# dnbaker/dashing

Measured on AMD Instinct MI355X. Metric: genome-pairs/sec, all-pairs HLL Jaccard (Ertl-MLE), N=10000 p=14, higher is better.
Workload: dtype u8/u32 popcount + f64 estimator; 1 GPU; BASELINE configs[2]: 10000 synthetic sketches, p=14 (16384 B each), all-pairs dist on MI355X; n_sketches=10000, p=14, k=31, estimator=ERTL_MLE

## Files before the change

dashing_amd/csrc/abi.hip:

```cpp
#include <algorithm>
#include <cstdlib>
#include <cstring>
#include <new>

#include "ctx.h"

using namespace dsh;

extern "C" {

const char *dsh_backend_name(void) { return "hip:gfx950"; }

int dsh_abi_version(void) { return DSH_ABI_VERSION; }

int dsh_device_count(void)
{
    int n = 0;
    if (hipGetDeviceCount(&n) != hipSuccess) return 0;
    return n;
}

static void release_ctx(dsh_ctx *c)
{
    (void)hipSetDevice(c->device);
// ... 476 lines not shown
    if (!c || !nparts_out) return DSH_EINVAL;
    const uint32_t k = (uint32_t)c->part_ready_ms.size();
    *nparts_out = k;
    if (k > cap && (ready_ms || floats)) return DSH_EINVAL;
    for (uint32_t q = 0; q < k; ++q) {
        if (ready_ms) ready_ms[q] = c->part_ready_ms[q];
        if (floats) floats[q] = c->part_floats[q];
    }
    return DSH_OK;
}

int dsh_finalize_phase_cycles(dsh_ctx *c, uint64_t *out16)
{
    if (!c || !out16) return DSH_EINVAL;
    int rc = bind(c);
    if (rc) return rc;
    if (!c->phase_cyc.ptr) return fail(c, DSH_ESTATE, "no call with the option finalize_timing yet");
    HIPCHK(c, hipStreamSynchronize(c->stream));
    HIPCHK(c, hipMemcpy(out16, c->phase_cyc.ptr, 16 * sizeof(uint64_t), hipMemcpyDeviceToHost));
    return DSH_OK;
}

int dsh_get_info(dsh_ctx *c, const char *name, int64_t *out)
{
    if (!c || !name || !out) return DSH_EINVAL;
    if (!std::strcmp(name, "planes")) *out = c->lay.P;
    else if (!std::strcmp(name, "vlo")) *out = c->lay.vlo;
    else if (!std::strcmp(name, "vhi")) *out = c->lay.vhi;
    else if (!std::strcmp(name, "threshold")) *out = c->lay.pbase + (int64_t)c->lay.P;
    else if (!std::strcmp(name, "pbase")) *out = c->lay.pbase;
    else if (!std::strcmp(name, "host_layout_us")) *out = (int64_t)c->host_layout_us;
    else if (!std::strcmp(name, "host_lists_us")) *out = (int64_t)c->host_lists_us;
    else if (!std::strcmp(name, "host_keys_wait_us")) *out = (int64_t)c->host_keys_wait_us;
    else if (!std::strcmp(name, "emax")) *out = c->emax;
    else if (!std::strcmp(name, "elow")) *out = c->elow;
    else if (!std::strcmp(name, "kc")) *out = c->kc;
    else if (!std::strcmp(name, "pair_groups")) *out = c->pair_groups;
    else if (!std::strcmp(name, "pair_round")) *out = c->pp.band_round.empty() ? 0 : c->pp.band_round[0];
    else if (!std::strcmp(name, "tile")) *out = kTile;
    else if (!std::strcmp(name, "parts_done")) *out = c->parts_done;
    else if (!std::strcmp(name, "parts_signalled")) *out = c->parts_signalled ? 1 : 0;
    else if (!std::strcmp(name, "sketch_kernel_us")) *out = (int64_t)(c->sketch_ms * 1000.0);
    else if (!std::strcmp(name, "fastx_decode_us")) *out = (int64_t)(c->fastx_ms * 1000.0);
    else if (!std::strcmp(name, "xch_recv_gated")) *out = c->xch.recv_gated ? 1 : 0;
    else if (!std::strcmp(name, "stats_route")) *out = c->gs.route_last;
    else if (!std::strcmp(name, "linkage_route")) *out = c->lk.route_last;
    else if (!std::strcmp(name, "mst_rounds")) *out = c->mst.rounds_last;
    else if (!std::strcmp(name, "mst_band_us")) *out = (int64_t)(c->mst.band_ms * 1000.0);
    else if (!std::strcmp(name, "place_kernel_us")) *out = (int64_t)(c->xch.place_ms * 1000.0);
    else if (!std::strcmp(name, "whatif_mfma")) {
#ifdef DSH_WHATIF_MFMA
        *out = 1;
#else
        *out = 0;
#endif
    }
    else if (!std::strcmp(name, "npad")) *out = c->lay.Npad;
    else if (!std::strcmp(name, "kpad")) *out = c->Kpad;
    else if (!std::strcmp(name, "cum_bytes")) *out = c->cum_bytes;
    else if (!std::strcmp(name, "sorted")) *out = c->lay.sorted;
    else if (!std::strcmp(name, "ncols")) *out = (int64_t)c->lay.ncols;
    else if (!std::strcmp(name, "lockstep")) *out = c->planes_valid && use_lockstep(c) ? 1 : 0;
    else if (!std::strcmp(name, "tiles")) *out = (int64_t)c->pp.T.size();
    else if (!std::strcmp(name, "bands")) *out = (int64_t)c->last_bands;
    else if (!std::strcmp(name, "items")) *out = (int64_t)c->pp.items.size();
    else if (!std::strcmp(name, "frag_items")) {
// ... 121 lines not shown
```

dashing_amd/csrc/ctx.h:

```cpp
#pragma once
#include <hip/hip_runtime.h>
#include <rccl/rccl.h>

#include <cstdarg>
#include <cstdio>
#include <cstdlib>
#include <deque>
#include <string>
#include <vector>

#include "../../include/dashing_hip.h"
#include "kernels.h"
#include "plan.h"

struct NoCopy {
    NoCopy() = default;
    NoCopy(const NoCopy &) = delete;
    NoCopy &operator=(const NoCopy &) = delete;
};

struct DevBuf : NoCopy {
    void *ptr = nullptr;
    size_t cap = 0;
    ~DevBuf() { release(); }
// ... 119 lines not shown
    Event ev_filled[2];
    Event ev_drained[2];
    bool drained_pending[2] = {false, false};
    unsigned out_turn = 0;
    std::deque<Event> tickets;
    uint64_t ticket_next = 0;
    Event ev_first_tiles;
    bool pass_from_zero = false;
    DevBuf hist;
    Event ev_keys;
    DevBuf cidx_rec, cidx_ent;
    uint32_t nbuckets = 0, ent_stride = 0;
    DevBuf colS_n, colS_key, colS_card, colS_th, colS_rl;
    uint32_t rl_stride = 0;
    dsh::plan::Layout lay;
    bool lay_built = false;
    dsh::plan::PairPlan pp;
    std::deque<Event> ev_part;
    uint32_t parts_done = 0;
    DevBuf sig;
    Staging st_sig;
    uint32_t sig_gen = 0;
    bool parts_signalled = false;
    int finalize_signal = -1;
    int can_wait_value = -1;
    int wall_clock_khz = 0;
    PinBuf pin_keys;
    const uint32_t *hk32 = nullptr;
    const uint32_t *hg32 = nullptr;
    const uint32_t *hv32 = nullptr;
    uint32_t pass_sparse_cap = 0;
    bool hk32_valid = false;
    double host_layout_us = 0, host_lists_us = 0, host_keys_wait_us = 0;
    Staging st_perm;
    DevBuf rowoff;
    Staging st_lists;
    uint32_t W = 0, Kpad = 0;
    int emax = 0, elow = 0, cum_bytes = 4;
    int kc = 16;
    int kc_opt = 0;
    int pair_groups = 3;
    int pair_groups_opt = 0;
    int emax_opt = -1;
    int elow_opt = -1;
    int part_band_tiles = 2048;
    int overflow_frag_permille = 500;
    int sparse_planes = -1;
    int sparse_cap = (int)dsh::plan::kSparseCapDefault;
    int sparse_sided = -1;
    int sparse_lds = 1;
    int sparse_run = 0;
    uint32_t sparse_run_used = 0;
    DevBuf sp_tab, sp_lists, sp_len, sp_slabs, sp_items;
    Staging st_sparse;
    std::vector<dsh::plan::U2> sp_have;
    uint64_t sp_serial = 0, lay_serial = 0;
    uint32_t sp_cap_have = 0;
    double sparse_ms = 0;
    std::vector<std::pair<hipEvent_t, hipEvent_t>> ev_sparse;
    int tail_bands = 2;
    std::vector<double> part_ready_ms;
    std::vector<uint64_t> part_floats;
    size_t last_bands = 0;
    uint64_t cum_budget = 8ull << 30;
    int sort_mode = -1;
    int range_sort_min_rows = 1024;
// ... 282 lines not shown
```

dashing_amd/csrc/engine.hip:

```cpp
#include <algorithm>
#include <chrono>
#include <cstring>

#include "ctx.h"

namespace dsh {

int prepare(dsh_ctx *c, int estim, int want_sorted, bool card_only, uint64_t want_rb, uint64_t want_re, uint32_t nparts,
            int rowsorted, const std::vector<uint64_t> *extra_in)
{
    static const std::vector<uint64_t> kNoExtra;
    std::vector<uint64_t> extra_cached;
    const std::vector<uint64_t> *extra = extra_in ? extra_in : &kNoExtra;
    if (!c->have_sketches) return fail(c, DSH_ESTATE, "no sketches loaded");
    if (estim < 0 || estim > 2) return fail(c, DSH_EINVAL, "bad estimator %d", estim);
    if (want_sorted < 0) {
        want_sorted = c->lay.sorted;
        want_rb = c->lay.rb;
        want_re = c->lay.re;
        rowsorted = 0;
        extra_cached = c->lay.extra;
        extra = &extra_cached;
    }
    if (!want_sorted) rowsorted = 0, extra = &kNoExtra;
// ... 165 lines not shown
                                         (size_t)(c->Kpad - K) * L.Npad * sizeof(uint32_t),
                                         c->stream));
            HIPCHK(c, launch_transform(c->stream, c->regs, L.ncols, c->p, L.pbase, L.P, c->W, L.Npad,
                                       (uint32_t *)c->planes.ptr,
                                       want_sorted ? (const uint32_t *)c->perm.ptr : nullptr));
        }
        c->aux_join_pending = true;
        c->lay_gen = c->pass_gen;
        c->planes_valid = true;
    }
    timer.stop(c->prep_ms, true);
    return DSH_OK;
}

namespace {

struct JobLayout {
    int want_sorted = 0;
    uint64_t lrb = 0, lre = 0;
    bool with_parts = false;
    bool with_extra = false;
};

struct PairRun {
    plan::Tuning tu;
    std::vector<uint64_t> item_off;
    plan::U4 *pinT = nullptr, *pinF = nullptr, *pinI = nullptr;
    bool signal = false;
    bool sig_upload = false;
    FinalizeLaunch fin{};
    hipEvent_t e_call0 = nullptr;
    std::vector<std::pair<size_t, hipEvent_t>> ev_part_t;
    std::vector<std::pair<hipEvent_t, hipEvent_t>> evp, evf;
};

JobLayout choose_layout(const dsh_ctx *c, const PairJob &job)
{
    JobLayout jl;
    const uint64_t jre = std::min<uint64_t>(job.row_end, c->n);
    const bool full_tri = !job.rect && job.row_begin == 0 && jre >= c->n;
    jl.with_parts = job.nparts > 0 && !job.rect && !job.sorted_rows;
    jl.lre = c->n;
    if (job.sorted_rows) jl.want_sorted = 1;
    else if (!job.rect && jre > job.row_begin &&
             (jl.with_parts || (c->sort_mode != 0 && (full_tri || jre - job.row_begin >= (uint64_t)c->range_sort_min_rows)))) {
        jl.want_sorted = 1;
        jl.lrb = job.row_begin;
        jl.lre = jre;
    }
    jl.with_extra = jl.want_sorted && jl.with_parts && !job.extra.empty() && jl.lre > jl.lrb;
    return jl;
}

constexpr uint64_t kSparseSlabBudget = 2ull << 30;
uint32_t sparse_list_stride(const dsh_ctx *c)
{
    return std::max<uint32_t>(8, (std::min<uint32_t>((uint32_t)c->sparse_cap, plan::kSparseCapMax) + 7) / 8 * 8);
}
int sparse_wordmajor(const dsh_ctx *c) { return c->sparse_lds && c->p <= 15 ? 1 : 0; }
uint32_t sparse_run_of(const dsh_ctx *c) { return c->sparse_run > 0 ? (uint32_t)c->sparse_run : plan::kSparseRunDefault; }
uint64_t sparse_slab_bytes(const dsh_ctx *c)
{
    return ((uint64_t)16 << c->p) + (uint64_t)kTile * sparse_list_stride(c) * sizeof(uint16_t) + kTile * sizeof(uint32_t);
}

plan::Tuning tuning_of(const dsh_ctx *c)
// ... 218 lines not shown
        f.a.sig = r.signal ? (uint32_t *)c->sig.ptr : nullptr;
        if (c->aux_join_pending) {
            HIPCHK(c, hipStreamWaitEvent(c->stream, c->ev_aux_join, 0));
            c->aux_join_pending = false;
        }
        HIPCHK(c, launch_finalize(fst, f));
        if (sg.part >= 0) {
            const size_t qp = (size_t)sg.part;
            while (c->ev_part.size() <= qp) HIPCHK(c, add_event(c->ev_part));
            HIPCHK(c, hipEventRecord(c->ev_part[qp], fst));
            c->parts_done = (uint32_t)qp + 1;
            if (r.e_call0) {
                hipEvent_t te = next_event(c);
                if (te) {
                    (void)hipEventRecord(te, fst);
                    r.ev_part_t.emplace_back(qp, te);
                }
            }
        }
    }
    return DSH_OK;
}

int read_profile(dsh_ctx *c, const PairRun &r)
{
    const plan::Layout &L = c->lay;
    HIPCHK(c, hipStreamSynchronize(c->stream));
    for (auto &e : r.evp) {
        float ms = 0;
        (void)hipEventElapsedTime(&ms, e.first, e.second);
        c->pair_ms += ms;
        if (c->Kpad) c->pair_launches++;
    }
    for (auto &e : r.evf) {
        float ms = 0;
        (void)hipEventElapsedTime(&ms, e.first, e.second);
        c->fin_ms += ms;
    }
    c->sparse_ms = 0;
    for (auto &e : c->ev_sparse) {
        float ms = 0;
        (void)hipEventElapsedTime(&ms, e.first, e.second);
        c->sparse_ms += ms;
    }
    c->ev_sparse.clear();
    auto fill_part_floats = [&] {
        for (size_t i = 0; i < c->part_floats.size(); ++i) {
            if (L.rowsorted && i + 1 < L.part_w.size()) c->part_floats[i] = L.rowoff_w[L.part_w[i + 1]] - L.rowoff_w[L.part_w[i]];
            else if (!L.rowsorted && L.extra.empty() && i + 1 < L.parts.size()) c->part_floats[i] = plan::tri_span(c->n, L.parts[i], L.parts[i + 1]);
            else if (!L.rowsorted) c->part_floats[i] = plan::rowset_span(c->n, L.rb, L.re, L.extra);
        }
    };
    if (r.signal && r.e_call0 && c->wall_clock_khz > 0) {
        std::vector<unsigned long long> st(kSigMaxParts + 1);
        HIPCHK(c, hipMemcpy(st.data(), (uint32_t *)c->sig.ptr + kSigPartTime, kSigMaxParts * sizeof(unsigned long long), hipMemcpyDeviceToHost));
        HIPCHK(c, hipMemcpy(&st[kSigMaxParts], (uint32_t *)c->sig.ptr + kSigT0, sizeof(unsigned long long), hipMemcpyDeviceToHost));
        c->part_ready_ms.assign(c->parts_done, 0.0);
        c->part_floats.assign(c->parts_done, 0);
        for (size_t i = 0; i < c->part_ready_ms.size(); ++i)
            c->part_ready_ms[i] = (double)(long long)(st[i] - st[kSigMaxParts]) / (double)c->wall_clock_khz;
        fill_part_floats();
    } else if (r.e_call0 && !r.ev_part_t.empty()) {
        c->part_ready_ms.assign(c->parts_done, 0.0);
        c->part_floats.assign(c->parts_done, 0);
        for (auto &pe : r.ev_part_t) {
            float ms = 0;
// ... 35 lines not shown
    if (job.k < 1) return fail(c, DSH_EINVAL, "bad k %d", job.k);
    const auto t_l0 = std::chrono::steady_clock::now();
    plan::PairPlan &pp = c->pp;
    plan::PairQuery q;
    q.rect = job.rect;
    q.sorted_rows = job.sorted_rows;
    q.want_parts = jl.with_parts;
    q.row_begin = job.row_begin;
    q.row_end = job.row_end;
    q.col_begin = job.col_begin;
    q.col_end = job.col_end;
    r.tu = tuning_of(c);
    if (!plan::build_tiles(c->lay, q, r.tu, pp)) {
        pp.T.clear();
        return DSH_OK;
    }
    c->last_bands = pp.bands.size();
    if ((rc = reserve_lists(c, r))) return rc;
    c->host_lists_us = std::chrono::duration<double, std::micro>(std::chrono::steady_clock::now() - t_l0).count();

    if (jl.with_parts && pp.nparts >= 1 && pp.nparts <= kSigMaxParts && !c->finalize_timing && !c->finalize_stop && c->finalize_signal != 0) {
        r.signal = device_can_wait_value(c);
        if (!r.signal && c->finalize_signal == 1) return fail(c, DSH_ENODEV, "option finalize_signal = 1, but the device does not support hipStreamWaitValue32");
    }
    c->parts_signalled = r.signal;
    if (r.signal && (rc = stage_signal_block(c, r))) return rc;
    if (c->finalize_timing) {
        HIPCHK(c, c->phase_cyc.ensure(16 * sizeof(unsigned long long)));
        HIPCHK(c, hipMemsetAsync(c->phase_cyc.ptr, 0, 16 * sizeof(unsigned long long), c->stream));
    }
    r.fin = finalize_invariants(c, job, jl.with_extra);
    c->ev_sparse.clear();
    c->sparse_run_used = 0;
    if (!pp.sp_items.empty() && (rc = prepare_sparse(c))) return rc;
    for (size_t bi = 0; bi < pp.bands.size(); ++bi) {
        const uint64_t nslots = (uint64_t)(pp.bands[bi].second - pp.bands[bi].first) * kTile * kTile;
        if ((rc = upload_band(c, r, bi))) return rc;
        hipEvent_t a = nullptr, b = nullptr, d = nullptr;
        if (c->profiling) {
            a = next_event(c);
            b = next_event(c);
            d = next_event(c);
            if (a) (void)hipEventRecord(a, c->stream);
        }
        if ((rc = launch_sparse_items(c, bi, nslots))) return rc;
        if ((rc = launch_tile_kernel(c, r, bi, nslots))) return rc;
        if (b) (void)hipEventRecord(b, c->stream);
        if (bi == 0) {
            HIPCHK(c, c->ev_first_tiles.ensure());
            HIPCHK(c, hipEventRecord(c->ev_first_tiles, c->stream));
        }
        r.fin.a.nslots = nslots;
        if ((rc = finalize_band(c, r, bi))) return rc;
        if (d) (void)hipEventRecord(d, c->stream);
        if (a && b && d) {
            r.evp.emplace_back(a, b);
            r.evf.emplace_back(b, d);
        }
    }
    if (r.signal) c->parts_done = pp.nparts;
    return c->profiling ? read_profile(c, r) : DSH_OK;
}

}
```

dashing_amd/csrc/host/plan_capi.cpp:

```cpp
#include <algorithm>
#include <cstdarg>
#include <cstdio>
#include <cstring>
#include <vector>

#include "../linkage.h"
#include "../mst.h"
#include "../plan.h"
#include "../sketch_plan.h"
#include "../uf.h"

using namespace dsh;
using namespace dsh::plan;

namespace {

struct SparseCheck {
    const uint32_t *gcnt = nullptr;
    int planes = 0;
    uint32_t cap = 0;
    uint32_t *routes = nullptr;
    uint64_t routes_cap = 0;
    const uint32_t *thr = nullptr;
    uint32_t thr_cap = 0;
    int sided = 0;
    uint32_t *routes6 = nullptr, *items5 = nullptr, *slabs3 = nullptr;
    uint64_t items_cap = 0, slabs_cap = 0;
};

struct Err {
    char *buf;
    size_t cap;
    int fail(const char *fmt, ...)
    {
        if (buf && cap) {
            va_list ap;
            va_start(ap, fmt);
            vsnprintf(buf, cap, fmt, ap);
            va_end(ap);
        }
        return -1;
    }
};

struct CheckJob {
    uint64_t n = 0;
    const uint32_t *keys = nullptr;
    int mode = 0, want_sorted = 0;
    uint64_t rb = 0, re = 0, cb = 0, ce = 0;
    uint32_t nparts = 1;
    int want_parts = 0, p = 0;
    uint64_t cum_budget = 0;
    int lockstep = 1, nsplit = 0, ls_item_chunks = 64;
    std::vector<uint64_t> extra;
    uint32_t round_items = 0;
    const SparseCheck *sc = nullptr;
    uint64_t *stats = nullptr;
    int stats_slots = 9;
    bool rowsorted = false;
    uint64_t lrb = 0, lre = 0;
// ... 7 lines not shown
        if (mode == 2) want_sorted = 1;
        lrb = 0, lre = n;
        if (want_sorted && mode == 0) lrb = rb, lre = re;
    }
    bool plan_parts() const { return want_parts && mode == 0 && want_sorted; }
    std::vector<std::pair<uint64_t, uint64_t>> wanted_segments() const
    {
        std::vector<std::pair<uint64_t, uint64_t>> wsegs;
        wanted_order(n, lrb, lre, &extra, wsegs, rowsorted);
        return wsegs;
    }
};

bool in_rows(const std::vector<std::pair<uint64_t, uint64_t>> &wsegs, uint64_t i)
{
    for (auto &w : wsegs)
        if (i >= w.first && i < w.second) return true;
    return false;
}

uint32_t chunks_per_plane(const Tuning &tu) { return tu.W >= (uint32_t)tu.kc ? tu.W / tu.kc : 1; }

void job_layout(const CheckJob &job, Layout &L)
{
    std::vector<uint64_t> parts;
    if (job.want_sorted && !job.rowsorted) range_parts(job.n, job.lrb, job.lre, std::max<uint32_t>(job.want_parts ? job.nparts : 1, 1), parts);
    const SparseCheck *sc = job.sc;
    const SketchWords words{job.keys, sc ? sc->gcnt : nullptr, sc ? sc->thr : nullptr, sc ? sc->thr_cap : 0};
    const LayoutQuery query{job.want_sorted, job.lrb, job.lre, &parts, job.rowsorted ? std::max<uint32_t>(job.nparts, 1) : 0,
                            job.extra.empty() ? nullptr : &job.extra};
    build_layout(job.n, words, query, L);
}

bool job_plan(const CheckJob &job, const Layout &L, Tuning &tu, PairQuery &q, PairPlan &pp)
{
    const uint64_t m = 1ull << job.p;
    tu.W = (uint32_t)std::max<uint64_t>(1, m / 32);
    tu.kc = tu.W >= 32 ? 32 : 16;
    tu.cum_bytes = job.p <= 15 ? 2 : 4;
    tu.cum_budget = job.cum_budget;
    tu.nsplit = job.nsplit;
    tu.lockstep = job.lockstep && tu.W >= (uint32_t)tu.kc;
    tu.ls_item_chunks = job.ls_item_chunks;
    if (job.round_items) tu.round_items = job.round_items;
    if (job.round_items > 512) tu.small_round_items = 512;
    tu.p = job.p;
    if (job.sc) tu.sparse_planes = job.sc->planes, tu.sparse_cap = job.sc->cap, tu.sparse_sided = job.sc->sided;
    q.rect = job.mode == 1;
    q.sorted_rows = job.mode == 2;
    q.want_parts = job.plan_parts();
    q.row_begin = job.rb;
    q.row_end = job.re;
    q.col_begin = job.cb;
    q.col_end = job.ce;
    return build_pairs(L, q, tu, pp);
}


int check_rowsorted(const CheckJob &job, const Layout &L, Err &E)
{
    const uint64_t n = job.n, lrb = job.lrb;
    const uint32_t *keys = job.keys;
    const auto wsegs = job.wanted_segments();
    uint64_t nw = 0, wspan = 0;
    for (auto &w : wsegs) nw += w.second - w.first, wspan += tri_span(n, w.first, w.second);
    auto skey = [&](uint32_t g) { return ((uint32_t)key_T(keys[g]) << 12) | ((uint32_t)key_L(keys[g]) << 6) | (uint32_t)key_hi(keys[g]); };
    for (auto &w : wsegs)
        for (uint64_t s = w.first - lrb + 1; s < w.second - lrb; ++s)
            if (skey(L.perm[s - 1]) > skey(L.perm[s])) return E.fail("row-sorted: a wanted segment is not one key-ordered run at %llu", (unsigned long long)s);
    if (L.part_w.empty() || L.part_w.front() != 0 || L.part_w.back() != nw) return E.fail("row-sorted: part cuts do not span the wanted rows");
    for (size_t q = 1; q + 1 < L.part_w.size(); ++q) {
        if (L.part_w[q] <= L.part_w[q - 1]) return E.fail("row-sorted: cut %zu at %llu", q, (unsigned long long)L.part_w[q]);
        uint64_t w0 = 0;
        bool ok = false;
        for (auto &w : wsegs) {
            if (L.part_w[q] >= w0 && L.part_w[q] < w0 + (w.second - w.first)) ok = (L.part_w[q] - w0) % kTile == 0;
            w0 += w.second - w.first;
        }
        if (!ok) return E.fail("row-sorted: cut %zu at %llu is not at a tile row of the wanted order", q, (unsigned long long)L.part_w[q]);
    }
    if (L.part_w.size() - 1 > std::max<uint32_t>(job.nparts, 1)) return E.fail("row-sorted: more parts than asked for");
    uint64_t acc = 0, w_ = 0;
    if (L.rowoff_w.size() != nw + 1) return E.fail("row-sorted: rowoff_w size");
    for (auto &w : wsegs)
        for (uint64_t s = w.first - lrb; s < w.second - lrb; ++s, ++w_) {
            if (s >= L.rowoff.size() || L.rowoff[s] != acc || L.rowoff_w[w_] != acc) return E.fail("row-sorted: rowoff[%llu]", (unsigned long long)s);
            acc += n - 1 - L.perm[s];
        }
// ... 584 lines not shown
int dshh_plan_digest(uint64_t n, const uint32_t *keys, const uint32_t *gcnt, const uint32_t *thr, uint32_t thr_cap, int mode, int want_sorted,
                     uint64_t rb, uint64_t re, uint64_t cb, uint64_t ce, uint32_t nparts, int want_parts, int p, uint64_t cum_budget, int lockstep,
                     int nsplit, int ls_item_chunks, uint32_t round_items, int sparse_planes, int sparse_sided, uint32_t sparse_cap,
                     const uint64_t *extra, uint32_t n_extra, uint64_t *digests, uint32_t digests_cap, uint64_t *features, char *err, size_t cap)
{
    Err E{err, cap};
    if (round_items % 256) return E.fail("round_items %u is not a multiple of 256", round_items);
    if (!digests || !features || digests_cap < kDigestSections || n_extra % 2) return E.fail("digests, features and whole extra segments are wanted");
    SparseCheck sc;
    sc.gcnt = gcnt;
    sc.planes = sparse_planes;
    sc.cap = sparse_cap;
    sc.thr = thr;
    sc.thr_cap = thr_cap;
    sc.sided = sparse_sided;
    CheckJob job = base_job(n, keys, mode, want_sorted, rb, re, nparts, want_parts, p, cum_budget);
    job.cb = cb, job.ce = ce;
    job.lockstep = lockstep, job.nsplit = nsplit, job.ls_item_chunks = ls_item_chunks;
    job.extra.assign(extra, extra + (extra ? n_extra : 0));
    job.round_items = round_items;
    job.sc = &sc;
    job.resolve();
    if (!job.extra.empty() && !(job.want_sorted && job.mode == 0)) return E.fail("extra segments need a sorted triangle layout");
    Layout L;
    job_layout(job, L);
    Tuning tu;
    PairQuery q;
    PairPlan pp;
    const bool any = job_plan(job, L, tu, q, pp);
    *features = digest_plan(L, tu, q, pp, any, digests);
    return (int)kDigestSections;
}

uint64_t dshh_sparse_table_fills(const uint32_t *items4, uint64_t n, uint32_t run)
{
    static_assert(sizeof(U4) == 4 * sizeof(uint32_t), "an item is four words");
    return sparse_table_fills(reinterpret_cast<const U4 *>(items4), (size_t)n, run);
}

uint64_t dshh_rowsorted_split(uint64_t n, uint64_t rb, uint64_t re) { return rowsorted_split(n, rb, re); }

int64_t dshh_threshold_bands(uint64_t n, uint64_t rb, uint64_t re, uint64_t ncols, uint64_t band_bytes, uint64_t row_cap,
                             uint64_t *bounds, uint64_t cap)
{
    const uint64_t band_floats = std::max<uint64_t>(band_bytes / sizeof(float), 1);
    if (!ncols && re > n) re = n;
    uint64_t nb = 0;
    if (cap) bounds[0] = rb;
    for (uint64_t b0 = rb; b0 < re;) {
        b0 = ncols ? std::min<uint64_t>(re, b0 + rect_band_rows(ncols, band_floats)) : tri_band_end(n, b0, re, band_floats, row_cap);
        if (++nb >= cap) return -1;
        bounds[nb] = b0;
    }
    return (int64_t)nb;
}

uint64_t dshh_hist_grid(uint64_t units, uint64_t lds_bytes, uint32_t cus, uint64_t *iters)
{
    const uint64_t grid = hist_grid(units, lds_bytes, cus);
    if (iters) *iters = units / (4 * grid) + (units % (4 * grid) ? 1 : 0);
    return grid;
}

int64_t dshh_greedy_bands(uint64_t n, uint64_t band_bytes, uint64_t row_cap, uint64_t *bounds, uint64_t cap)
{
    const uint64_t band_floats = std::max<uint64_t>(band_bytes / sizeof(float), 1);
// ... 252 lines not shown
```

dashing_amd/csrc/plan.cpp:

```cpp
#include "plan.h"

#include <algorithm>
#include <cstring>

namespace dsh {
namespace plan {

uint64_t tri_index(uint64_t n, uint64_t i, uint64_t j) { return i * (2 * n - i - 1) / 2 + j - (i + 1); }

uint64_t tri_span(uint64_t n, uint64_t rb, uint64_t re)
{
    if (re > n) re = n;
    if (rb >= re) return 0;
    const uint64_t cnt = re - rb;
    return cnt * (n - 1) - (rb + re - 1) * cnt / 2;
}

uint64_t tri_band_end(uint64_t n, uint64_t b0, uint64_t re, uint64_t band_floats, uint64_t row_cap)
{
    const uint64_t max_rows = std::min<uint64_t>(std::max<uint64_t>(row_cap, 1), kBandMaxRows);
    uint64_t b1 = b0, span = 0;
    do {
        span += n - 1 - b1;
        ++b1;
// ... 808 lines not shown

static void cut_segments(const Layout &L, PairPlan &pp)
{
    const std::vector<size_t> &pstart = pp.part_first;
    pp.segs.resize(pp.bands.size());
    for (size_t bi = 0; bi < pp.bands.size(); ++bi) {
        size_t b = pp.bands[bi].first;
        while (b < pp.bands[bi].second) {
            const size_t q = part_of_tile(pstart, b);
            const size_t e = std::min(pp.bands[bi].second, pstart[q + 1]);
            const bool last_of_part = e == pstart[q + 1];
            Seg sg{b, e, pp.nparts && last_of_part ? (int)q : -1, 1};
            for (size_t t = b; t < e; ++t) {
                int lo, hi;
                tile_vrange(L, pp.T[t], lo, hi);
                sg.hist_bins = std::max(sg.hist_bins, hi - lo + 1);
            }
            pp.segs[bi].push_back(sg);
            b = e;
        }
    }
}

static void order_tiles(const Tuning &tu, PairPlan &pp)
{
    pp.rank.resize(pp.T.size());
    for (auto &sv : pp.segs)
        for (auto &sg : sv)
            for (size_t t = sg.b; t < sg.e; ++t) pp.rank[t] = (uint32_t)(t - sg.b);
    for (auto &sv : pp.segs)
        for (auto &sg : sv) xcd_order(pp.T, pp.rank, sg.b, sg.e, tu.lockstep ? 2 : 1);
}

static void order_sparse_items(const std::vector<U4> &T, const std::pair<size_t, size_t> &bd, uint32_t NT, size_t first, size_t last, std::vector<U4> &sp_items)
{
    if (last - first <= 1) return;
    auto table_block = [&](const U4 &it) { return it.y & kSpItemTransposed ? T[bd.first + it.x].x : T[bd.first + it.x].y; };
    constexpr size_t nx = 8;
    std::vector<uint32_t> per_col(NT, 0), cols;
    for (size_t k = first; k < last; ++k) per_col[table_block(sp_items[k])]++;
    for (uint32_t b = 0; b < NT; ++b)
        if (per_col[b]) cols.push_back(b);
    std::stable_sort(cols.begin(), cols.end(), [&](uint32_t a, uint32_t b) { return per_col[a] > per_col[b]; });
    std::vector<uint32_t> xcd_of(NT, 0);
    size_t load[nx] = {0};
    for (uint32_t b : cols) {
        size_t x = 0;
        for (size_t y = 1; y < nx; ++y)
            if (load[y] < load[x]) x = y;
        xcd_of[b] = (uint32_t)x;
        load[x] += per_col[b];
    }
    std::vector<U4> lists[nx];
    for (size_t k = first; k < last; ++k) lists[xcd_of[table_block(sp_items[k])]].push_back(sp_items[k]);
    for (auto &l : lists)
        std::stable_sort(l.begin(), l.end(), [&](const U4 &a, const U4 &b) {
            const U4 &ta = T[bd.first + a.x], &tb = T[bd.first + b.x];
            const uint32_t ca = table_block(a), cb = table_block(b), pa = a.y & kSpPlaneMask, pb = b.y & kSpPlaneMask;
            return ca != cb ? ca < cb : pa != pb ? pa > pb : ta.x + ta.y < tb.x + tb.y;
        });
    size_t q = first;
    for (size_t r = 0; q < last; ++r)
        for (size_t x = 0; x < nx; ++x)
            if (r < lists[x].size()) sp_items[q++] = lists[x][r];
}

uint64_t sparse_table_fills(const U4 *items, size_t n, uint32_t run)
{
    if (run == 0) return 0;
    uint64_t fills = 0;
    for (size_t x = 0; x < 8 && x < n; ++x) {
        uint32_t have = 0;
        size_t i = 0;
        for (size_t k = x; k < n; k += 8, i = i + 1 == run ? 0 : i + 1) {
            const uint32_t ts = items[k].y & kSpItemTransposed ? items[k].z : items[k].w;
            if (i == 0 || ts != have) fills += 4;
            have = ts;
        }
    }
    return fills;
}

static void route_sparse(const Layout &L, const Tuning &tu, const SparseGate &gate, PairPlan &pp)
{
    const std::vector<U4> &T = pp.T;
    const uint32_t NT = L.Npad / kTile;
    pp.sp.assign(T.size(), 0);
    pp.spb.assign(T.size(), 0);
    pp.sided_items = pp.transposed_items = pp.table_slabs = 0;
    pp.band_sp_items.assign(pp.bands.size(), std::make_pair((size_t)0, (size_t)0));
    if (!gate.any()) return;
    pp.slab_of.assign((size_t)NT * std::max<uint32_t>(L.P, 1), -1);
    std::vector<uint8_t> listed;
    auto slab = [&](uint32_t b, uint32_t pl, bool lists) -> uint32_t {
        int32_t &s = pp.slab_of[(size_t)b * L.P + pl];
        if (s < 0) {
            s = (int32_t)pp.slabs.size();
            pp.slabs.push_back(U2{b, pl | (gate.sided_can && sided_polarity(L, b, L.pbase + 1 + (int)pl) ? kSpSlabA : 0u)});
            listed.push_back(0);
        }
        if (lists) listed[(size_t)s] = 1;
        return (uint32_t)s;
    };
    for (size_t bi = 0; bi < pp.bands.size(); ++bi) {
        const auto &bd = pp.bands[bi];
        const size_t i0 = pp.sp_items.size();
        uint64_t band_planes = 0;
        for (size_t t = bd.first; t < bd.second; ++t) band_planes += T[t].w - T[t].z;
        const Route route = gate.route_for(band_planes);
        for (size_t t = bd.first; t < bd.second && route != Route::None; ++t) {
            uint32_t below, above;
            tile_route(L, gate, route, T[t], below, above);
            const uint32_t k = below + above;
            if (!k || pp.slabs.size() + 2 * k > tu.sparse_max_slabs) continue;
            pp.sp[t] = (uint8_t)above;
            pp.spb[t] = (uint8_t)below;
            for (uint32_t x = 0; x < k; ++x) {
                const uint32_t pl = x < above ? T[t].w - 1 - x : T[t].z + (x - above);
                bool tr = false;
                bool both = true;
                uint32_t fl = 0;
                if (route == Route::Sided) {
                    const int v = L.pbase + 1 + (int)pl;
                    tr = T[t].x != T[t].y && sided_depth(L, T[t].y, v) > sided_depth(L, T[t].x, v);
                    both = T[t].x == T[t].y;
                    const uint32_t lb = tr ? T[t].y : T[t].x, tb = tr ? T[t].x : T[t].y;
                    fl = (sided_polarity(L, lb, v) ? kSpItemListA : 0u) | (sided_polarity(L, tb, v) ? kSpItemTabA : 0u) | (tr ? kSpItemTransposed : 0u);
                    ++pp.sided_items;
                    pp.transposed_items += tr;
                }
                pp.sp_items.push_back(U4{(uint32_t)(t - bd.first), pl | fl, slab(T[t].x, pl, both || !tr), slab(T[t].y, pl, both || tr)});
            }
        }
        order_sparse_items(T, bd, NT, i0, pp.sp_items.size(), pp.sp_items);
        pp.band_sp_items[bi] = std::make_pair(i0, pp.sp_items.size());
    }
    for (size_t k = 0; k < pp.slabs.size(); ++k)
        if (!listed[k]) pp.slabs[k].y |= kSpSlabTableOnly, ++pp.table_slabs;
}

static void chunk_ranges(const Tuning &tu, PairPlan &pp)
{
    const std::vector<U4> &T = pp.T;
    const uint32_t KC = (uint32_t)tu.kc;
    const uint32_t cpp = tu.W >= KC ? tu.W / KC : 1;
    std::vector<U2> &CR = pp.chunks;
    CR.resize(T.size());
    if (tu.W >= KC) {
        for (size_t t = 0; t < T.size(); ++t) CR[t] = U2{(T[t].z + pp.spb[t]) * cpp, (T[t].w - pp.sp[t]) * cpp};
    } else {
        for (size_t t = 0; t < T.size(); ++t)
            CR[t] = U2{(uint32_t)(((uint64_t)T[t].z * tu.W) / KC), (uint32_t)(((uint64_t)T[t].w * tu.W + KC - 1) / KC)};
    }
    for (auto &bd : pp.bands) pp.max_band = std::max(pp.max_band, bd.second - bd.first);
}

bool build_tiles(const Layout &L, const PairQuery &job, const Tuning &tu, PairPlan &pp)
{
    pp.T.clear();
    pp.bands.clear();
    pp.band_items.clear();
    pp.segs.clear();
    pp.items.clear();
    pp.band_frags.clear();
    pp.band_round.clear();
    pp.sp.clear();
    pp.spb.clear();
    pp.sp_items.clear();
    pp.band_sp_items.clear();
    pp.slabs.clear();
    pp.nparts = 0;
    pp.max_band = 0;
    std::vector<size_t> trow_first;
    std::vector<uint64_t> trow_w;
    if (!list_tiles(L, job, pp.T, trow_first, trow_w)) return false;
    uint64_t job_planes = 0;
    for (const U4 &t : pp.T) job_planes += t.w - t.z;
    const SparseGate gate = sparse_gate(L, job, tu, job_planes);
    part_starts(L, job, trow_first, trow_w, pp);
    cut_bands(L, tu, tail_cuts(L, tu, gate, pp), pp);
    cut_segments(L, pp);
    order_tiles(tu, pp);
    route_sparse(L, tu, gate, pp);
    chunk_ranges(tu, pp);
    return true;
}

static void overflow_fragments(const Tuning &tu, uint64_t RI, uint32_t cpp, uint64_t piece, uint64_t ni, uint64_t &over, uint32_t &f)
{
    over = 0;
    f = 1;
    if (!tu.lockstep || tu.nsplit != 0 || RI == 0 || tu.overflow_frag_max_permille == 0 || piece != cpp || cpp < 2 || ni == 0) return;
    const uint64_t o = ni % RI;
    if (o == 0 || o * 1000 > RI * tu.overflow_frag_max_permille) return;
    uint32_t ff = 1;
    while (ff * 2 <= cpp && o * (ff * 2) <= RI) ff *= 2;
    if (ff < 2) return;
    over = o;
    f = ff;
}

static uint32_t band_round_items(const Tuning &tu, uint64_t ni)
{
// ... 64 lines not shown
            if (b0 >= CR[t].y) continue;
            const uint32_t len = (uint32_t)std::min<uint64_t>(CR[t].y - b0, piece);
            const U4 it{(uint32_t)(t - bd.first), (uint32_t)b0, (uint32_t)b0 + len, 0};
            if (place) out[first[piece - len]++] = it;
            else *out++ = it;
        }
        if (!by_length && tu.lockstep && lmin != lmax)
            std::stable_sort(I.begin() + g0, I.end(), [](const U4 &x, const U4 &y) { return x.z - x.y > y.z - y.y; });
    }
    uint64_t over = 0;
    uint32_t f = 1;
    const uint32_t RI = band_round_items(tu, I.size() - i0);
    overflow_fragments(tu, RI, cpp, piece, I.size() - i0, over, f);
    if (pp.band_round.size() <= bi) pp.band_round.resize(bi + 1, 0);
    pp.band_round[bi] = RI;
    if (pp.band_frags.size() <= bi) pp.band_frags.resize(bi + 1, 0);
    pp.band_frags[bi] = 0;
    if (over) {
        std::vector<U4> &tail = pp.sort_tmp;
        tail.assign(I.end() - (ptrdiff_t)over, I.end());
        I.resize(I.size() - over);
        const uint32_t fr = cpp / f;
        for (const U4 &it : tail)
            for (uint32_t b0 = it.y; b0 < it.z; b0 += fr) I.push_back(U4{it.x, b0, std::min<uint32_t>(it.z, b0 + fr), 1});
        pp.band_frags[bi] = (uint32_t)(over * f);
    }
    if (pp.band_items.size() <= bi) pp.band_items.resize(bi + 1);
    pp.band_items[bi] = std::make_pair(i0, I.size());
}

bool build_pairs(const Layout &L, const PairQuery &q, const Tuning &t, PairPlan &pp)
{
    if (!build_tiles(L, q, t, pp)) return false;
    for (size_t bi = 0; bi < pp.bands.size(); ++bi) build_band_items(t, pp, bi);
    return true;
}

void emit_tile_lists(const Layout &L, const PairPlan &pp, U4 *pinT, U4 *pinF)
{
    for (size_t bi = 0; bi < pp.bands.size(); ++bi) emit_band_lists(L, pp, bi, pinT, pinF);
}

void emit_band_lists(const Layout &L, const PairPlan &pp, size_t bi, U4 *pinT, U4 *pinF)
{
    const std::vector<U4> &T = pp.T;
    const size_t b0 = pp.bands[bi].first;
    for (const Seg &sg : pp.segs[bi])
        for (size_t t = sg.b; t < sg.e; ++t) {
            int lo, hi;
            tile_vrange(L, T[t], lo, hi);
            const uint32_t pl = T[t].z | (T[t].w << 8);
            pinT[t] = U4{T[t].x, T[t].y, pl, (uint32_t)lo | ((uint32_t)hi << 8)};
            const size_t at = sg.b + pp.rank[t];
            const uint32_t part = pp.nparts ? (uint32_t)part_of_tile(pp.part_first, t) : 0u;
            pinF[at] = U4{T[t].x, T[t].y, pl | ((uint32_t)lo << 16) | ((uint32_t)hi << 24), (uint32_t)(t - b0) | (part << 16)};
        }
}

uint64_t band_item_count(const Tuning &tu, const PairPlan &pp, size_t bi)
{
    const auto &bd = pp.bands[bi];
    const BandShape shape = band_shape(tu, pp, bi);
    uint64_t cnt = 0;
    for (size_t t = bd.first; t < bd.second; ++t) cnt += pieces_of(pp.chunks[t].y - pp.chunks[t].x, shape.piece);
    uint64_t over = 0;
    uint32_t f = 1;
// ... 124 lines not shown
```

dashing_amd/csrc/plan.h:

```cpp
#pragma once
#include <stddef.h>
#include <stdint.h>

#include <algorithm>
#include <utility>
#include <vector>

#include "consts.h"

namespace dsh {
namespace plan {

struct U4 { uint32_t x, y, z, w; };
struct U2 { uint32_t x, y; };

inline int key_lo(uint32_t k) { return (int)(k & 63u); }
inline int key_L(uint32_t k) { return (int)((k >> 6) & 63u); }
inline int key_T(uint32_t k) { return (int)((k >> 12) & 63u); }
inline int key_hi(uint32_t k) { return (int)((k >> 18) & 63u); }
inline bool key_bad(uint32_t k) { return (k & 0x80000000u) != 0; }

uint64_t tri_index(uint64_t n, uint64_t i, uint64_t j);
uint64_t tri_span(uint64_t n, uint64_t rb, uint64_t re);
void partition_rows(uint64_t n, uint32_t nparts, uint32_t align, uint64_t *bounds);
// ... 130 lines not shown
    int p = 0;
};

struct Seg {
    size_t b, e;
    int part;
    int hist_bins;
};

struct PairPlan {
    std::vector<U4> T;
    std::vector<std::pair<size_t, size_t>> bands;
    std::vector<std::pair<size_t, size_t>> band_items;
    std::vector<uint32_t> band_round;
    std::vector<std::vector<Seg>> segs;
    std::vector<U4> items;
    std::vector<uint32_t> band_frags;
    std::vector<uint32_t> rank;
    std::vector<U2> chunks;
    uint64_t per_tile_bytes = 0;
    size_t max_band = 0;
    uint32_t nparts = 0;
    std::vector<uint32_t> part_tiles;
    std::vector<size_t> part_first;
    std::vector<uint32_t> sort_first;
    std::vector<U4> sort_tmp;
    std::vector<uint8_t> sp;
    std::vector<uint8_t> spb;
    std::vector<U4> sp_items;
    uint64_t sided_items = 0, transposed_items = 0, table_slabs = 0;
    std::vector<std::pair<size_t, size_t>> band_sp_items;
    std::vector<U2> slabs;
    std::vector<int32_t> slab_of;
};
uint32_t sparse_bound(const Layout &L, uint32_t b, int v);
int sided_depth(const Layout &L, uint32_t b, int v);
int sided_polarity(const Layout &L, uint32_t b, int v);

bool build_pairs(const Layout &L, const PairQuery &q, const Tuning &t, PairPlan &pp);
bool build_tiles(const Layout &L, const PairQuery &q, const Tuning &t, PairPlan &pp);
void build_band_items(const Tuning &t, PairPlan &pp, size_t band);
void emit_tile_lists(const Layout &L, const PairPlan &pp, U4 *tiles_out, U4 *ftiles_out);
void emit_band_lists(const Layout &L, const PairPlan &pp, size_t band, U4 *tiles_out, U4 *ftiles_out);
uint64_t band_item_count(const Tuning &t, const PairPlan &pp, size_t band);

}
}
```

Before: 4.590 billion pairs/s.

## Defer sparse item emission behind first tile launch and radix-sort sparse items

Splits sparse planning into slab assignment (in build_tiles) and a separate emit_sparse_items pass. The engine now emits and uploads sparse items after the first band's tile kernel is queued, so host work overlaps GPU execution. The comparison-based stable sorts in order_sparse_items are replaced with counting and radix passes over packed keys, using scratch buffers kept in PairPlan. This adds bookkeeping that subtracts the build time from the pair timing, plus a test entry point that needs to match the old ordering.

```diff
diff --git a/dashing_amd/csrc/abi.hip b/dashing_amd/csrc/abi.hip
--- a/dashing_amd/csrc/abi.hip
+++ b/dashing_amd/csrc/abi.hip
@@ -532,6 +532,7 @@
     else if (!std::strcmp(name, "host_layout_us")) *out = (int64_t)c->host_layout_us;
     else if (!std::strcmp(name, "host_lists_us")) *out = (int64_t)c->host_lists_us;
     else if (!std::strcmp(name, "host_keys_wait_us")) *out = (int64_t)c->host_keys_wait_us;
+    else if (!std::strcmp(name, "host_sparse_us")) *out = (int64_t)c->host_sparse_us;
     else if (!std::strcmp(name, "emax")) *out = c->emax;
     else if (!std::strcmp(name, "elow")) *out = c->elow;
     else if (!std::strcmp(name, "kc")) *out = c->kc;
diff --git a/dashing_amd/csrc/ctx.h b/dashing_amd/csrc/ctx.h
--- a/dashing_amd/csrc/ctx.h
+++ b/dashing_amd/csrc/ctx.h
@@ -175,6 +175,7 @@
     uint32_t pass_sparse_cap = 0;
     bool hk32_valid = false;
     double host_layout_us = 0, host_lists_us = 0, host_keys_wait_us = 0;
+    double host_sparse_us = 0;
     Staging st_perm;
     DevBuf rowoff;
     Staging st_lists;
diff --git a/dashing_amd/csrc/engine.hip b/dashing_amd/csrc/engine.hip
--- a/dashing_amd/csrc/engine.hip
+++ b/dashing_amd/csrc/engine.hip
@@ -221,6 +221,7 @@
     hipEvent_t e_call0 = nullptr;
     std::vector<std::pair<size_t, hipEvent_t>> ev_part_t;
     std::vector<std::pair<hipEvent_t, hipEvent_t>> evp, evf;
+    double build_in_pair_ms = 0;
 };
 
 JobLayout choose_layout(const dsh_ctx *c, const PairJob &job)
@@ -505,6 +506,7 @@
         c->pair_ms += ms;
         if (c->Kpad) c->pair_launches++;
     }
+    c->pair_ms -= r.build_in_pair_ms;
     for (auto &e : r.evf) {
         float ms = 0;
         (void)hipEventElapsedTime(&ms, e.first, e.second);
@@ -606,7 +608,7 @@
     r.fin = finalize_invariants(c, job, jl.with_extra);
     c->ev_sparse.clear();
     c->sparse_run_used = 0;
-    if (!pp.sp_items.empty() && (rc = prepare_sparse(c))) return rc;
+    c->host_sparse_us = 0;
     for (size_t bi = 0; bi < pp.bands.size(); ++bi) {
         const uint64_t nslots = (uint64_t)(pp.bands[bi].second - pp.bands[bi].first) * kTile * kTile;
         if ((rc = upload_band(c, r, bi))) return rc;
@@ -617,13 +619,21 @@
             d = next_event(c);
             if (a) (void)hipEventRecord(a, c->stream);
         }
-        if ((rc = launch_sparse_items(c, bi, nslots))) return rc;
         if ((rc = launch_tile_kernel(c, r, bi, nslots))) return rc;
-        if (b) (void)hipEventRecord(b, c->stream);
         if (bi == 0) {
             HIPCHK(c, c->ev_first_tiles.ensure());
             HIPCHK(c, hipEventRecord(c->ev_first_tiles, c->stream));
         }
+        if (bi == 0 && pp.sp_count) {
+            const auto t_s0 = std::chrono::steady_clock::now();
+            plan::emit_sparse_items(c->lay, pp);
+            c->host_sparse_us = std::chrono::duration<double, std::micro>(std::chrono::steady_clock::now() - t_s0).count();
+            const double prep0 = c->prep_ms;
+            if ((rc = prepare_sparse(c))) return rc;
+            r.build_in_pair_ms = c->prep_ms - prep0;
+        }
+        if ((rc = launch_sparse_items(c, bi, nslots))) return rc;
+        if (b) (void)hipEventRecord(b, c->stream);
         r.fin.a.nslots = nslots;
         if ((rc = finalize_band(c, r, bi))) return rc;
         if (d) (void)hipEventRecord(d, c->stream);
diff --git a/dashing_amd/csrc/host/plan_capi.cpp b/dashing_amd/csrc/host/plan_capi.cpp
--- a/dashing_amd/csrc/host/plan_capi.cpp
+++ b/dashing_amd/csrc/host/plan_capi.cpp
@@ -26,6 +26,7 @@
     int sided = 0;
     uint32_t *routes6 = nullptr, *items5 = nullptr, *slabs3 = nullptr;
     uint64_t items_cap = 0, slabs_cap = 0;
+    uint32_t max_slabs = 0;
 };
 
 struct Err {
@@ -99,7 +100,7 @@
     build_layout(job.n, words, query, L);
 }
 
-bool job_plan(const CheckJob &job, const Layout &L, Tuning &tu, PairQuery &q, PairPlan &pp)
+bool job_plan(const CheckJob &job, const Layout &L, Tuning &tu, PairQuery &q, PairPlan &pp, bool two_step = false)
 {
     const uint64_t m = 1ull << job.p;
     tu.W = (uint32_t)std::max<uint64_t>(1, m / 32);
@@ -113,6 +114,7 @@
     if (job.round_items > 512) tu.small_round_items = 512;
     tu.p = job.p;
     if (job.sc) tu.sparse_planes = job.sc->planes, tu.sparse_cap = job.sc->cap, tu.sparse_sided = job.sc->sided;
+    if (job.sc && job.sc->max_slabs) tu.sparse_max_slabs = job.sc->max_slabs;
     q.rect = job.mode == 1;
     q.sorted_rows = job.mode == 2;
     q.want_parts = job.plan_parts();
@@ -120,7 +122,14 @@
     q.row_end = job.re;
     q.col_begin = job.cb;
     q.col_end = job.ce;
-    return build_pairs(L, q, tu, pp);
+    if (!two_step) return build_pairs(L, q, tu, pp);
+    if (!build_tiles(L, q, tu, pp)) return false;
+    for (size_t bi = 0; bi < pp.bands.size(); ++bi) {
+        if (bi == 1) emit_sparse_items(L, pp);
+        build_band_items(tu, pp, bi);
+    }
+    if (pp.bands.size() < 2) emit_sparse_items(L, pp);
+    return true;
 }
 
 
@@ -771,6 +780,56 @@
     return (int)kDigestSections;
 }
 
+int dshh_plan_sparse_items(uint64_t n, const uint32_t *keys, const uint32_t *gcnt, const uint32_t *thr, uint32_t thr_cap, uint64_t rb, uint64_t re,
+                           uint32_t nparts, int want_parts, int p, uint64_t cum_budget, uint32_t round_items, int sparse_planes, int sparse_sided,
+                           uint32_t sparse_cap, uint32_t sparse_max_slabs, int two_step, uint64_t *counts, uint32_t *tiles6, uint64_t tiles_cap,
+                           uint64_t *bands4, uint64_t bands_cap, uint32_t *items4, uint64_t items_cap, uint32_t *slabs2, uint64_t slabs_cap,
+                           uint32_t *chunks2, char *err, size_t cap)
+{
+    Err E{err, cap};
+    if (round_items == 0 || round_items % 256) return E.fail("round_items %u is not a positive multiple of 256", round_items);
+    if (!counts || !tiles6 || !bands4 || !items4 || !slabs2 || !chunks2) return E.fail("every list is wanted");
+    SparseCheck sc;
+    sc.gcnt = gcnt;
+    sc.planes = sparse_planes;
+    sc.cap = sparse_cap;
+    sc.thr = thr;
+    sc.thr_cap = thr_cap;
+    sc.sided = sparse_sided;
+    sc.max_slabs = sparse_max_slabs;
+    CheckJob job = base_job(n, keys, 0, 1, rb, re, nparts, want_parts, p, cum_budget);
+    job.round_items = round_items;
+    job.sc = &sc;
+    job.resolve();
+    Layout L;
+    job_layout(job, L);
+    Tuning tu;
+    PairQuery q;
+    PairPlan pp;
+    for (int i = 0; i < 9; ++i) counts[i] = 0;
+    counts[8] = L.Npad / kTile;
+    if (!job_plan(job, L, tu, q, pp, two_step != 0)) return 0;
+    counts[0] = pp.T.size(), counts[1] = pp.bands.size(), counts[2] = pp.sp_items.size(), counts[3] = pp.slabs.size();
+    counts[4] = pp.sided_items, counts[5] = pp.transposed_items, counts[6] = pp.table_slabs, counts[7] = pp.items.size();
+    if (pp.T.size() > tiles_cap || pp.bands.size() > bands_cap || pp.sp_items.size() > items_cap || pp.slabs.size() > slabs_cap)
+        return E.fail("%zu tiles, %zu bands, %zu items, %zu slabs: no room", pp.T.size(), pp.bands.size(), pp.sp_items.size(), pp.slabs.size());
+    for (size_t t = 0; t < pp.T.size(); ++t) {
+        uint32_t *o = tiles6 + 6 * t;
+        o[0] = pp.T[t].x, o[1] = pp.T[t].y, o[2] = pp.T[t].z, o[3] = pp.T[t].w, o[4] = pp.spb[t], o[5] = pp.sp[t];
+        chunks2[2 * t] = pp.chunks[t].x, chunks2[2 * t + 1] = pp.chunks[t].y;
+    }
+    for (size_t bi = 0; bi < pp.bands.size(); ++bi) {
+        uint64_t *o = bands4 + 4 * bi;
+        o[0] = pp.bands[bi].first, o[1] = pp.bands[bi].second, o[2] = pp.band_sp_items[bi].first, o[3] = pp.band_sp_items[bi].second;
+    }
+    for (size_t k = 0; k < pp.sp_items.size(); ++k) {
+        uint32_t *o = items4 + 4 * k;
+        o[0] = pp.sp_items[k].x, o[1] = pp.sp_items[k].y, o[2] = pp.sp_items[k].z, o[3] = pp.sp_items[k].w;
+    }
+    for (size_t k = 0; k < pp.slabs.size(); ++k) slabs2[2 * k] = pp.slabs[k].x, slabs2[2 * k + 1] = pp.slabs[k].y;
+    return 0;
+}
+
 uint64_t dshh_sparse_table_fills(const uint32_t *items4, uint64_t n, uint32_t run)
 {
     static_assert(sizeof(U4) == 4 * sizeof(uint32_t), "an item is four words");
diff --git a/dashing_amd/csrc/plan.cpp b/dashing_amd/csrc/plan.cpp
--- a/dashing_amd/csrc/plan.cpp
+++ b/dashing_amd/csrc/plan.cpp
@@ -864,37 +864,70 @@
         for (auto &sg : sv) xcd_order(pp.T, pp.rank, sg.b, sg.e, tu.lockstep ? 2 : 1);
 }
 
-static void order_sparse_items(const std::vector<U4> &T, const std::pair<size_t, size_t> &bd, uint32_t NT, size_t first, size_t last, std::vector<U4> &sp_items)
-{
-    if (last - first <= 1) return;
-    auto table_block = [&](const U4 &it) { return it.y & kSpItemTransposed ? T[bd.first + it.x].x : T[bd.first + it.x].y; };
+struct SpKeyRange {
+    uint32_t pmin = ~0u, pmax = 0, smin = ~0u, smax = 0;
+};
+static void order_sparse_items(uint32_t NT, size_t first, size_t last, const SpKeyRange &kr, PairPlan &pp)
+{
+    const size_t n = last - first;
+    if (n <= 1) return;
     constexpr size_t nx = 8;
-    std::vector<uint32_t> per_col(NT, 0), cols;
-    for (size_t k = first; k < last; ++k) per_col[table_block(sp_items[k])]++;
+    std::vector<PairPlan::SpRec> &ra = pp.sp_rec_a, &rb = pp.sp_rec_b;
+    std::vector<uint32_t> &cnt = pp.sp_cnt, &per_col = pp.sp_per_col, &cols = pp.sp_cols, &by_count = pp.sp_cols_tmp, &brank = pp.sp_brank;
+    per_col.assign(NT, 0);
+    for (size_t k = 0; k < n; ++k) ++per_col[ra[k].key >> 40];
+    cols.clear();
+    uint32_t maxc = 0;
     for (uint32_t b = 0; b < NT; ++b)
-        if (per_col[b]) cols.push_back(b);
-    std::stable_sort(cols.begin(), cols.end(), [&](uint32_t a, uint32_t b) { return per_col[a] > per_col[b]; });
-    std::vector<uint32_t> xcd_of(NT, 0);
-    size_t load[nx] = {0};
-    for (uint32_t b : cols) {
+        if (per_col[b]) cols.push_back(b), maxc = std::max(maxc, per_col[b]);
+    cnt.assign((size_t)maxc + 1, 0);
+    for (uint32_t b : cols) ++cnt[maxc - per_col[b] + 1];
+    for (size_t v = 1; v <= maxc; ++v) cnt[v] += cnt[v - 1];
+    by_count.resize(cols.size());
+    for (uint32_t b : cols) by_count[cnt[maxc - per_col[b]]++] = b;
+    brank.resize(NT);
+    size_t load[nx] = {0}, nblk[nx] = {0}, at[nx];
+    for (uint32_t b : by_count) {
         size_t x = 0;
         for (size_t y = 1; y < nx; ++y)
             if (load[y] < load[x]) x = y;
-        xcd_of[b] = (uint32_t)x;
+        brank[b] = (uint32_t)x;
         load[x] += per_col[b];
-    }
-    std::vector<U4> lists[nx];
-    for (size_t k = first; k < last; ++k) lists[xcd_of[table_block(sp_items[k])]].push_back(sp_items[k]);
-    for (auto &l : lists)
-        std::stable_sort(l.begin(), l.end(), [&](const U4 &a, const U4 &b) {
-            const U4 &ta = T[bd.first + a.x], &tb = T[bd.first + b.x];
-            const uint32_t ca = table_block(a), cb = table_block(b), pa = a.y & kSpPlaneMask, pb = b.y & kSpPlaneMask;
-            return ca != cb ? ca < cb : pa != pb ? pa > pb : ta.x + ta.y < tb.x + tb.y;
-        });
-    size_t q = first;
-    for (size_t r = 0; q < last; ++r)
+        ++nblk[x];
+    }
+    at[0] = 0;
+    for (size_t x = 1; x < nx; ++x) at[x] = at[x - 1] + nblk[x - 1];
+    for (uint32_t b : cols) brank[b] = (uint32_t)at[brank[b]]++;
+    const uint64_t srange = (uint64_t)kr.smax - kr.smin + 1, prange = (uint64_t)kr.pmax - kr.pmin + 1;
+    auto pass = [&](std::vector<PairPlan::SpRec> &src, std::vector<PairPlan::SpRec> &dst, size_t nb, auto digit) {
+        cnt.assign(nb + 1, 0);
+        for (size_t k = 0; k < n; ++k) ++cnt[digit(src[k].key) + 1];
+        for (size_t v = 1; v <= nb; ++v) cnt[v] += cnt[v - 1];
+        dst.resize(n);
+        for (size_t k = 0; k < n; ++k) dst[cnt[digit(src[k].key)]++] = src[k];
+    };
+    const uint32_t pmax = kr.pmax, smin = kr.smin;
+    auto d_s = [&](uint64_t key) { return (size_t)((uint32_t)key - smin); };
+    auto d_p = [&](uint64_t key) { return (size_t)(pmax - (uint32_t)((key >> 32) & 0xFFu)); };
+    if (srange * prange <= (1u << 16)) {
+        pass(ra, rb, (size_t)(srange * prange), [&](uint64_t key) { return d_p(key) * (size_t)srange + d_s(key); });
+    } else {
+        pass(ra, rb, (size_t)srange, d_s);
+        pass(rb, ra, (size_t)prange, d_p);
+        ra.swap(rb);
+    }
+    pass(rb, ra, cols.size(), [&](uint64_t key) { return (size_t)brank[key >> 40]; });
+    size_t off[nx];
+    off[0] = 0;
+    for (size_t x = 1; x < nx; ++x) off[x] = off[x - 1] + load[x - 1];
+    std::vector<U4> &tmp = pp.sort_tmp;
+    tmp.resize(n);
+    U4 *I = pp.sp_items.data() + first;
+    size_t q = 0;
+    for (size_t r = 0; q < n; ++r)
         for (size_t x = 0; x < nx; ++x)
-            if (r < lists[x].size()) sp_items[q++] = lists[x][r];
+            if (r < load[x]) tmp[q++] = I[ra[off[x] + r].idx];
+    std::copy(tmp.begin(), tmp.end(), I);
 }
 
 uint64_t sparse_table_fills(const U4 *items, size_t n, uint32_t run)
@@ -920,26 +953,23 @@
     pp.sp.assign(T.size(), 0);
     pp.spb.assign(T.size(), 0);
     pp.sided_items = pp.transposed_items = pp.table_slabs = 0;
+    pp.sp_count = 0;
     pp.band_sp_items.assign(pp.bands.size(), std::make_pair((size_t)0, (size_t)0));
+    pp.band_route.assign(pp.bands.size(), (uint8_t)Route::None);
     if (!gate.any()) return;
     pp.slab_of.assign((size_t)NT * std::max<uint32_t>(L.P, 1), -1);
-    std::vector<uint8_t> listed;
-    auto slab = [&](uint32_t b, uint32_t pl, bool lists) -> uint32_t {
+    auto slab = [&](uint32_t b, uint32_t pl) {
         int32_t &s = pp.slab_of[(size_t)b * L.P + pl];
-        if (s < 0) {
-            s = (int32_t)pp.slabs.size();
-            pp.slabs.push_back(U2{b, pl | (gate.sided_can && sided_polarity(L, b, L.pbase + 1 + (int)pl) ? kSpSlabA : 0u)});
-            listed.push_back(0);
-        }
-        if (lists) listed[(size_t)s] = 1;
-        return (uint32_t)s;
+        if (s >= 0) return;
+        s = (int32_t)pp.slabs.size();
+        pp.slabs.push_back(U2{b, pl | (gate.sided_can && sided_polarity(L, b, L.pbase + 1 + (int)pl) ? kSpSlabA : 0u)});
     };
     for (size_t bi = 0; bi < pp.bands.size(); ++bi) {
         const auto &bd = pp.bands[bi];
-        const size_t i0 = pp.sp_items.size();
         uint64_t band_planes = 0;
         for (size_t t = bd.first; t < bd.second; ++t) band_planes += T[t].w - T[t].z;
         const Route route = gate.route_for(band_planes);
+        pp.band_route[bi] = (uint8_t)route;
         for (size_t t = bd.first; t < bd.second && route != Route::None; ++t) {
             uint32_t below, above;
             tile_route(L, gate, route, T[t], below, above);
@@ -947,12 +977,44 @@
             if (!k || pp.slabs.size() + 2 * k > tu.sparse_max_slabs) continue;
             pp.sp[t] = (uint8_t)above;
             pp.spb[t] = (uint8_t)below;
+            pp.sp_count += k;
+            for (uint32_t x = 0; x < k; ++x) {
+                const uint32_t pl = x < above ? T[t].w - 1 - x : T[t].z + (x - above);
+                slab(T[t].x, pl);
+                slab(T[t].y, pl);
+            }
+        }
+    }
+}
+
+void emit_sparse_items(const Layout &L, PairPlan &pp)
+{
+    const std::vector<U4> &T = pp.T;
+    const uint32_t NT = L.Npad / kTile;
+    pp.sp_items.clear();
+    pp.sided_items = pp.transposed_items = pp.table_slabs = 0;
+    pp.band_sp_items.assign(pp.bands.size(), std::make_pair((size_t)0, (size_t)0));
+    if (!pp.sp_count) return;
+    pp.sp_items.reserve(pp.sp_count);
+    std::vector<uint8_t> &listed = pp.sp_listed;
+    listed.assign(pp.slabs.size(), 0);
+    std::vector<PairPlan::SpRec> &rec = pp.sp_rec_a;
+    for (size_t bi = 0; bi < pp.bands.size(); ++bi) {
+        const auto &bd = pp.bands[bi];
+        const size_t i0 = pp.sp_items.size();
+        const bool sided = pp.band_route[bi] == (uint8_t)Route::Sided;
+        SpKeyRange kr;
+        rec.clear();
+        for (size_t t = bd.first; t < bd.second && pp.band_route[bi] != (uint8_t)Route::None; ++t) {
+            const uint32_t above = pp.sp[t], k = above + pp.spb[t];
+            const uint32_t s = T[t].x + T[t].y;
+            if (k) kr.smin = std::min(kr.smin, s), kr.smax = std::max(kr.smax, s);
             for (uint32_t x = 0; x < k; ++x) {
                 const uint32_t pl = x < above ? T[t].w - 1 - x : T[t].z + (x - above);
                 bool tr = false;
                 bool both = true;
                 uint32_t fl = 0;
-                if (route == Route::Sided) {
+                if (sided) {
                     const int v = L.pbase + 1 + (int)pl;
                     tr = T[t].x != T[t].y && sided_depth(L, T[t].y, v) > sided_depth(L, T[t].x, v);
                     both = T[t].x == T[t].y;
@@ -961,14 +1023,21 @@
                     ++pp.sided_items;
                     pp.transposed_items += tr;
                 }
-                pp.sp_items.push_back(U4{(uint32_t)(t - bd.first), pl | fl, slab(T[t].x, pl, both || !tr), slab(T[t].y, pl, both || tr)});
+                const uint32_t si = (uint32_t)pp.slab_of[(size_t)T[t].x * L.P + pl], sj = (uint32_t)pp.slab_of[(size_t)T[t].y * L.P + pl];
+                if (both || !tr) listed[si] = 1;
+                if (both || tr) listed[sj] = 1;
+                rec.push_back(PairPlan::SpRec{(uint64_t)(tr ? T[t].x : T[t].y) << 40 | (uint64_t)pl << 32 | s, (uint32_t)(pp.sp_items.size() - i0)});
+                kr.pmin = std::min(kr.pmin, pl), kr.pmax = std::max(kr.pmax, pl);
+                pp.sp_items.push_back(U4{(uint32_t)(t - bd.first), pl | fl, si, sj});
             }
         }
-        order_sparse_items(T, bd, NT, i0, pp.sp_items.size(), pp.sp_items);
+        order_sparse_items(NT, i0, pp.sp_items.size(), kr, pp);
         pp.band_sp_items[bi] = std::make_pair(i0, pp.sp_items.size());
     }
-    for (size_t k = 0; k < pp.slabs.size(); ++k)
+    for (size_t k = 0; k < pp.slabs.size(); ++k) {
+        pp.slabs[k].y &= ~kSpSlabTableOnly;
         if (!listed[k]) pp.slabs[k].y |= kSpSlabTableOnly, ++pp.table_slabs;
+    }
 }
 
 static void chunk_ranges(const Tuning &tu, PairPlan &pp)
@@ -1001,6 +1070,8 @@
     pp.sp_items.clear();
     pp.band_sp_items.clear();
     pp.slabs.clear();
+    pp.band_route.clear();
+    pp.sp_count = 0;
     pp.nparts = 0;
     pp.max_band = 0;
     std::vector<size_t> trow_first;
@@ -1131,6 +1202,7 @@
 bool build_pairs(const Layout &L, const PairQuery &q, const Tuning &t, PairPlan &pp)
 {
     if (!build_tiles(L, q, t, pp)) return false;
+    emit_sparse_items(L, pp);
     for (size_t bi = 0; bi < pp.bands.size(); ++bi) build_band_items(t, pp, bi);
     return true;
 }
diff --git a/dashing_amd/csrc/plan.h b/dashing_amd/csrc/plan.h
--- a/dashing_amd/csrc/plan.h
+++ b/dashing_amd/csrc/plan.h
@@ -186,6 +186,12 @@
     std::vector<std::pair<size_t, size_t>> band_sp_items;
     std::vector<U2> slabs;
     std::vector<int32_t> slab_of;
+    uint64_t sp_count = 0;
+    std::vector<uint8_t> band_route;
+    struct SpRec { uint64_t key; uint32_t idx; };
+    std::vector<uint8_t> sp_listed;
+    std::vector<uint32_t> sp_cnt, sp_per_col, sp_cols, sp_cols_tmp, sp_brank;
+    std::vector<SpRec> sp_rec_a, sp_rec_b;
 };
 uint32_t sparse_bound(const Layout &L, uint32_t b, int v);
 int sided_depth(const Layout &L, uint32_t b, int v);
@@ -194,6 +200,7 @@
 bool build_pairs(const Layout &L, const PairQuery &q, const Tuning &t, PairPlan &pp);
 bool build_tiles(const Layout &L, const PairQuery &q, const Tuning &t, PairPlan &pp);
 void build_band_items(const Tuning &t, PairPlan &pp, size_t band);
+void emit_sparse_items(const Layout &L, PairPlan &pp);
 void emit_tile_lists(const Layout &L, const PairPlan &pp, U4 *tiles_out, U4 *ftiles_out);
 void emit_band_lists(const Layout &L, const PairPlan &pp, size_t band, U4 *tiles_out, U4 *ftiles_out);
 uint64_t band_item_count(const Tuning &t, const PairPlan &pp, size_t band);
```

New measurement: 4.793 billion pairs/s, median of 6. +4.4%, better.
